# CarbonMatrixLab/AbX

Measured on AMD Instinct MI355X. Metric: diffusion-steps/sec (100 samples, ~350-res complex), higher is better.
Workload: dtype f32; 1 GPU; L352: L=352 (Lab 228 + antigen 124), 100 samples of one complex over 1 GPU(s), 1 step = ScoreNetwork (3 passes) + get_prev + reverse, seeded random weights, ESM off; L=352, samples_total=100, chunk=auto, parallelism=sample-shard x1, no collective in the step

## Files before the change

### abx_amd/csrc/gemm_as.hip

```cpp
#include <stdlib.h>

#include <type_traits>

#include "common.h"
#include "abx_hip.h"

namespace {

typedef __attribute__((address_space(3))) void* lds_ptr_t;
typedef const __attribute__((address_space(1))) void* glb_ptr_t;

constexpr int AS_BM = 64, AS_BN = 128, AS_NK = 12, AS_RING = 3;
constexpr int AS_KT = 4096;
constexpr int AS_A = AS_NK * AS_KT;
constexpr int AS_STAGE = 2 * AS_BN * 32;
constexpr int AS_HALF = AS_KT / 2;
constexpr int AS_OFF_RING = AS_A;
constexpr int AS_OFF_ST = AS_OFF_RING + AS_RING * AS_STAGE;
constexpr int AS_OFF_CONST = AS_OFF_ST + 4 * 64 * 4;
constexpr int AS_LDS = AS_OFF_CONST + 2 * 1024;

__device__ __forceinline__ void as_glds16(const void* src, char* dst_wave_base) {
    __builtin_amdgcn_global_load_lds((glb_ptr_t)src, (lds_ptr_t)dst_wave_base, 16, 0, 0);
}
// ... 552 lines not shown

constexpr int AD_BN = 192, AD_NK2 = 12, AD_NK1 = 8, AD_NS = AD_NK2 + AD_NK1;
constexpr int AD_PLANE = AD_BN * 32;
constexpr int AD_STAGE = 2 * AD_PLANE;
constexpr int AD_OFF_RING = AS_A;
constexpr int AD_OFF_ST = AD_OFF_RING + 2 * AD_STAGE;
constexpr int AD_OFF_CONST = AD_OFF_ST + 4 * 64 * 4;
constexpr int AD_LDS = AD_OFF_CONST + 4 * AD_BN * 4;
static_assert(AD_LDS <= 81920, "two blocks per CU");
constexpr int AD_P0 = 4;
constexpr int ad_wslot(int t) { return t < 4 ? AD_OFF_RING + (t & 1) * AD_STAGE : ((t - 4) % 3 == 0 ? AD_OFF_RING : ((t - 4) % 3 == 1 ? 0 : AD_OFF_RING + AD_STAGE)); }

__device__ __forceinline__ void ad_issue_z(const AbxGemm& g, char* lds, int m0, int b, int wm) {
    const int lane = threadIdx.x & 63;
    const bool remap = g.pair_Lp > 0;
    const long long row0 = remap ? 0 : m0;
    const char* baseA = reinterpret_cast<const char*>(g.A2 + (long long)b * g.sA2b + row0 * g.sA2m);
    unsigned offA[2];
#pragma unroll
    for (int i = 0; i < 2; ++i) {
        const int r = 16 * i + (lane >> 2), p = lane & 3;
        const int kq = p ^ ((r >> 2) & 3);
        const int gri = min(m0 + wm * 32 + r, g.M - 1);
        long long gr = gri;
        if (remap) {
            const int pi = gri / g.pair_Lp, pj = min(gri - pi * g.pair_Lp, g.pair_L - 1);
            gr = (long long)pi * g.pair_L + pj;
        }
        offA[i] = (unsigned)(((gr - row0) * g.sA2m + kq * 4) * 4);
    }
    char* dst = lds + wm * AS_HALF;
#pragma unroll
    for (int kt = 0; kt < AD_NK2; ++kt)
#pragma unroll
        for (int i = 0; i < 2; ++i) as_glds16(baseA + kt * 64 + as_vgpr32(offA[i]), dst + kt * AS_KT + i * 1024);
}

template <bool FIRST>
__device__ __forceinline__ void ad_conv_ptile(AsConv& c, char* img) {
    const int lane = threadIdx.x & 63, r = lane & 31, h = lane >> 5;
    float xv[8];
#pragma unroll
    for (int e = 0; e < 8; ++e) xv[e] = *reinterpret_cast<const float*>(img + (8 * h + e) * 128 + r * 4);
    as_conv_values<FIRST>(c, xv, img);
}

__device__ __forceinline__ void ad_rendezvous(u32x4 (&fa)[2], u32x4 (&fb)[3][2]) {
    asm volatile("s_waitcnt lgkmcnt(0)\n\ts_barrier"
                 : "+v"(fa[0]), "+v"(fa[1]), "+v"(fb[0][0]), "+v"(fb[0][1]), "+v"(fb[1][0]), "+v"(fb[1][1]), "+v"(fb[2][0]), "+v"(fb[2][1])
                 :
                 : "memory");
}
template <int N>
__device__ __forceinline__ void ad_rendezvous_vm(u32x4 (&fa)[2], u32x4 (&fb)[3][2]) {
    asm volatile("s_waitcnt vmcnt(%8) lgkmcnt(0)\n\ts_barrier"
                 : "+v"(fa[0]), "+v"(fa[1]), "+v"(fb[0][0]), "+v"(fb[0][1]), "+v"(fb[1][0]), "+v"(fb[1][1]), "+v"(fb[2][0]), "+v"(fb[2][1])
                 : "n"(N)
                 : "memory");
}

template <bool EDGE>
__device__ __forceinline__ void as_dual_block(const AbxGemm& g, char* lds, int mt, int b) {
    const int lane = threadIdx.x & 63, wave = __builtin_amdgcn_readfirstlane(threadIdx.x >> 6);
    const int wm = wave >> 1, wn = wave & 1, h = lane >> 5;
    const int m0 = mt * AS_BM;
    float* st = reinterpret_cast<float*>(lds + AD_OFF_ST);
    const float* cc = reinterpret_cast<const float*>(lds + AD_OFF_CONST);

    const char* wbase2 = reinterpret_cast<const char*>(g.B2_split);
    const char* wbase1 = reinterpret_cast<const char*>(g.B_split + (long long)b * g.sB3b);
    const long long wk2 = g.sB23k * 2, wk1 = g.sB3k * 2;
    const unsigned wchunk2 = (unsigned)(32 * g.sB23n * 2), wchunk1 = (unsigned)(32 * g.sB3n * 2);
    unsigned woff2, woff1;
    {
        const int row = lane >> 1, half = (lane & 1) ^ ((row >> 3) & 1);
        woff2 = (unsigned)((wm * g.sB23p + (long long)row * g.sB23n + 8 * half) * 2);
        woff1 = (unsigned)((wm * g.sB3p + (long long)row * g.sB3n + 8 * half) * 2);
    }
    auto issue_w = [&](auto s_) __attribute__((always_inline)) {
        constexpr int s = decltype(s_)::value;
        char* dst = lds + ad_wslot(s) + wm * AD_PLANE;
        if constexpr (s < AD_NK2) {
            const char* src = wbase2 + s * wk2;
#pragma unroll
            for (int i = 0; i < 6; ++i) as_glds16(src + i * wchunk2 + as_vgpr32(woff2), dst + i * 1024);
        } else {
            const char* src = wbase1 + (s - AD_NK2) * wk1;
#pragma unroll
            for (int i = 0; i < 6; ++i) as_glds16(src + i * wchunk1 + as_vgpr32(woff1), dst + i * 1024);
        }
    };

    const char* pbase = reinterpret_cast<const char*>(g.A + (long long)b * g.sAb + m0);
    const long long pk = 16LL * g.sAk * 4;
    unsigned poff[2];
#pragma unroll
    for (int i = 0; i < 2; ++i) {
        const int kl = 8 * i + (lane >> 3);
        const int gm = min(m0 + wm * 32 + 4 * (lane & 7), g.M - 4) - m0;
        poff[i] = (unsigned)(((long long)kl * g.sAk + gm) * 4);
    }
    auto issue_p = [&](int kt) __attribute__((always_inline)) {
        char* dst = lds + (AD_P0 + kt) * AS_KT + wm * AS_HALF;
        const char* src = pbase + kt * pk;
#pragma unroll
        for (int i = 0; i < 2; ++i) as_glds16(src + as_vgpr32(poff[i]), dst + i * 1024);
    };

    const float cs2 = __builtin_ldexpf(1.0f, -ABX_F16_A_EXP - g.b2_exp), inv_cs2 = __builtin_ldexpf(1.0f, ABX_F16_A_EXP + g.b2_exp);
    const float cs1 = __builtin_ldexpf(1.0f, -ABX_F16_A_EXP - g.b_exp), inv_cs1 = __builtin_ldexpf(1.0f, ABX_F16_A_EXP + g.b_exp);
    AsConv cz, cp;
    char* a_half = lds + wm * AS_HALF;
    if (wn == 0) {
        ad_issue_z(g, lds, m0, b, wm);
        as_conv_init(cz, g);
        cz.ln = true;
        cz.relu = false;
        cp = cz;
        as_wait_vm<20>();
        as_conv_ktile<true>(cz, a_half);
        as_conv_ktile<false>(cz, a_half + AS_KT);
    } else {
        const float* c0 = wm ? g.ln_csum : g.ln2_csum;
        const float* c1 = wm ? g.bias : g.bias2;
#pragma unroll
        for (int a = 0; a < 2; ++a)
#pragma unroll
            for (int i = 0; i < 3; ++i) {
                char* dst = lds + AD_OFF_CONST + (2 * wm + a) * (AD_BN * 4) + i * 256;
                __builtin_amdgcn_global_load_lds((glb_ptr_t)((a ? c1 : c0) + i * 64 + lane), (lds_ptr_t)dst, 4, 0, 0);
            }
        issue_w(IC<0>{});
        issue_w(IC<1>{});
        as_wait_vm<6>();
    }
    __syncthreads();

    const int offAf = wm * AS_HALF + as_plane_off<32>(0, lane & 31, h);
    const int offBf = as_plane_off<AD_BN>(0, wn * 96 + (lane & 31), h);
    u32x4 fa[2][2], fb[2][3][2];
    auto read_frags = [&](int set, int kt, int wslot) __attribute__((always_inline)) {
#pragma unroll
        for (int p = 0; p < 2; ++p) fa[set][p] = *reinterpret_cast<const u32x4*>(lds + kt * AS_KT + offAf + p * 1024);
#pragma unroll
        for (int j = 0; j < 3; ++j)
#pragma unroll
            for (int p = 0; p < 2; ++p) fb[set][j][p] = *reinterpret_cast<const u32x4*>(lds + offBf + wslot + p * AD_PLANE + j * 1024);
    };

    f32x16 gatev[3], acc[3];
    const float* st_w = st + wm * 32 + 4 * h;
    auto gate_values = [&]() __attribute__((always_inline)) {
#pragma unroll
        for (int j = 0; j < 3; ++j) {
            const int n = wn * 96 + j * 32 + (lane & 31);
            const float csum2 = cc[n] * inv_cs2, bias2 = cc[AD_BN + n];
#pragma unroll
            for (int rq = 0; rq < 4; ++rq) {
                const f32x4 dm4 = *reinterpret_cast<const f32x4*>(st_w + 8 * rq), rs4 = *reinterpret_cast<const f32x4*>(st_w + 64 + 8 * rq);
#pragma unroll
                for (int c = 0; c < 4; ++c) {
                    const float gv = rs4[c] * (gatev[j][4 * rq + c] - dm4[c] * csum2) + bias2;
                    gatev[j][4 * rq + c] = sigmoidf_(gv);
                }
            }
        }
    };

    f32x4 rv[4][3];
    long long row_off_c[4];
    bool row_ok[4];
    auto load_resid = [&]() __attribute__((always_inline)) {
        const float* rd = g.resid + (long long)b * g.sRb;
#pragma unroll
        for (int rq = 0; rq < 4; ++rq) {
            const int m = m0 + wm * 32 + 8 * rq + 4 * h + (lane & 3);
            bool ok = !EDGE || m < g.M;
            long long mo = m;
            if (g.c_pair) {
                const int pi = m / g.pair_Lp, pj = m - pi * g.pair_Lp;
                ok = ok && pj < g.pair_L;
                mo = (long long)pi * g.pair_L + pj;
            }
            row_ok[rq] = ok;
            row_off_c[rq] = mo * g.sCm;
#pragma unroll
            for (int j = 0; j < 3; ++j) {
                const int n = wn * 96 + j * 32 + ((lane & 31) >> 2) * 4;
                rv[rq][j] = (f32x4){0.f, 0.f, 0.f, 0.f};
                if (ok) rv[rq][j] = *reinterpret_cast<const f32x4*>(rd + mo * g.sRm + n);
            }
        }
    };

    auto step = [&](auto s_, auto role_) __attribute__((always_inline)) {
        constexpr int s = decltype(s_)::value, role = decltype(role_)::value, set = s & 1;
        if constexpr (role == 0) ad_rendezvous(fa[set], fb[set]);
        else ad_rendezvous_vm<(s >= 3 && s + 2 < AD_NS) ? 6 : 0>(fa[set], fb[set]);
        if constexpr (role == 1) {
            if constexpr (s < 2) issue_w(IC<s + 2>{});
            else if constexpr (s == 2) { issue_w(IC<4>{}); issue_w(IC<5>{}); }
            else if constexpr (s + 3 < AD_NS) issue_w(IC<s + 3>{});
        } else {
            constexpr int np = s < AD_P0 ? 0 : (s - AD_P0 + 1 < AD_NK1 ? s - AD_P0 + 1 : AD_NK1);
            if constexpr (s >= AD_P0 && s < AD_P0 + AD_NK1) issue_p(s - AD_P0);
            if constexpr (s < AD_NK2 - 2) {
                as_wait_vm<(24 - 2 * (s + 3)) + 2 * np>();
                as_conv_ktile<false>(cz, a_half + (s + 2) * AS_KT);
                if constexpr (s == AD_NK2 - 3) as_conv_finish(cz, st, wm, g.ln_eps, cs2);
            } else if constexpr (s < AD_NK2) {
                as_wait_vm<2 * (np - 1 - (s - 10))>();
                ad_conv_ptile<s == 10>(cp, a_half + (AD_P0 + s - 10) * AS_KT);
            } else if constexpr (s - AD_NK2 + 2 < AD_NK1) {
                constexpr int kp = s - AD_NK2 + 2;
                as_wait_vm<2 * (AD_NK1 - 1 - kp)>();
                ad_conv_ptile<false>(cp, a_half + (AD_P0 + kp) * AS_KT);
                if constexpr (kp == AD_NK1 - 1) as_conv_finish(cp, st + 128, wm, g.ln_eps, cs1, 1.0f / (float)(AD_NK1 * 16));
            }
        }
        if constexpr (s + 1 < AD_NS) read_frags((s + 1) & 1, (s + 1) < AD_NK2 ? s + 1 : s + 1 - AD_NK2 + AD_P0, ad_wslot(s + 1));
        u32x4 p2[3];
#pragma unroll
        for (int j = 0; j < 3; ++j) p2[j] = f16x8_lo(fb[set][j][0]);
        if constexpr (s < AD_NK2) {
            if constexpr (s == 0) {
                const f32x16 z = {0.f, 0.f, 0.f, 0.f, 0.f, 0.f, 0.f, 0.f, 0.f, 0.f, 0.f, 0.f, 0.f, 0.f, 0.f, 0.f};
#pragma unroll
                for (int j = 0; j < 3; ++j) gatev[j] = mfma_split(fa[set][1], p2[j], z);
            } else {
#pragma unroll
                for (int j = 0; j < 3; ++j) gatev[j] = mfma_split(fa[set][1], p2[j], gatev[j]);
            }
#pragma unroll
            for (int j = 0; j < 3; ++j) gatev[j] = mfma_split(fa[set][0], fb[set][j][1], gatev[j]);
#pragma unroll
            for (int j = 0; j < 3; ++j) gatev[j] = mfma_split(fa[set][0], fb[set][j][0], gatev[j]);
        } else {
            if constexpr (s == AD_NK2) {
                const f32x16 z = {0.f, 0.f, 0.f, 0.f, 0.f, 0.f, 0.f, 0.f, 0.f, 0.f, 0.f, 0.f, 0.f, 0.f, 0.f, 0.f};
#pragma unroll
                for (int j = 0; j < 3; ++j) acc[j] = mfma_split(fa[set][1], p2[j], z);
            } else {
#pragma unroll
                for (int j = 0; j < 3; ++j) acc[j] = mfma_split(fa[set][1], p2[j], acc[j]);
            }
#pragma unroll
            for (int j = 0; j < 3; ++j) acc[j] = mfma_split(fa[set][0], fb[set][j][1], acc[j]);
#pragma unroll
            for (int j = 0; j < 3; ++j) acc[j] = mfma_split(fa[set][0], fb[set][j][0], acc[j]);
        }
        if constexpr (s == AD_NK2) gate_values();
    };

    read_frags(0, 0, ad_wslot(0));
    auto walk = [&](auto role_) __attribute__((always_inline)) { as_static_for<0, AD_NS>([&](auto s_) { step(s_, role_); }); };
    if (wn == 0) walk(IC<0>{});
    else walk(IC<1>{});

    float* Cb = g.C + (long long)b * g.sCb;
    bool bad = false;
    load_resid();
#pragma unroll
    for (int j = 0; j < 3; ++j) {
        const int nl = wn * 96 + j * 32 + (lane & 31);
        const float csum1 = cc[2 * AD_BN + nl] * inv_cs1, bias1 = cc[3 * AD_BN + nl];
        const int n = wn * 96 + j * 32 + ((lane & 31) >> 2) * 4;
#pragma unroll
        for (int rq = 0; rq < 4; ++rq) {
            const f32x4 dm4 = *reinterpret_cast<const f32x4*>(st_w + 128 + 8 * rq), rs4 = *reinterpret_cast<const f32x4*>(st_w + 192 + 8 * rq);
            float x[4], o[4];
#pragma unroll
            for (int c = 0; c < 4; ++c) {
                float v = rs4[c] * (acc[j][4 * rq + c] - dm4[c] * csum1);
                v = v + bias1;
                x[c] = v * gatev[j][4 * rq + c];
            }
            as_quad_transpose(x, o);
            f32x4 ov;
#pragma unroll
            for (int c = 0; c < 4; ++c) {
                ov[c] = o[c] + rv[rq][j][c];
                bad |= row_ok[rq] && __builtin_amdgcn_classf(ov[c], 0x207);
            }
            if (row_ok[rq]) *reinterpret_cast<f32x4*>(Cb + row_off_c[rq] + n) = ov;
        }
    }
    if (g.range_flag && __any(bad) && lane == 0) atomicOr(g.range_flag, g.range_tag);
}

__global__ __launch_bounds__(256, 2) void gemm_as_dual_kernel(const AbxGemm g) {
    extern __shared__ __attribute__((aligned(16))) float as_smem[];
    char* lds = reinterpret_cast<char*>(as_smem);
    const ClockProbe probe(g.clock_probe);
    const unsigned ntm = (unsigned)((g.M + AS_BM - 1) / AS_BM);
    const unsigned nwg = gridDim.x, bid = blockIdx.x;
    const unsigned q = nwg >> 3, r = nwg & 7, xcd = bid & 7, loc = bid >> 3;
    const unsigned wgid = (xcd < r ? xcd * (q + 1) : r * (q + 1) + (xcd - r) * q) + loc;
    const int b = (int)(wgid / ntm), mt = (int)(wgid - (unsigned)b * ntm);
    if ((mt + 1) * AS_BM > g.M) as_dual_block<true>(g, lds, mt, b);
    else as_dual_block<false>(g, lds, mt, b);
    probe.finish();
}

int as_dual_dispatch(const AbxGemm& g, hipStream_t st, int* rc) {
    auto al16 = [](const void* p) { return (reinterpret_cast<uintptr_t>(p) & 15) == 0; };
    static const bool off = [] {
        const char* e = getenv("ABX_NO_DUAL_AS");
        return e != nullptr && !(e[0] == '0' && e[1] == 0);
    }();
    if (off) return 1;
    if (g.exact == 1 || g.K != AD_NK1 * 16 || g.K2 != AD_NK2 * 16 || g.N != AD_BN) return 1;
    if (!g.A || g.A_split || g.sAm != 1 || g.M % 4 != 0 || g.M < 4 || !g.B_split || !g.B2_split || !g.b_f16) return 1;
    if (!g.ln_csum || g.ln_stats || !g.ln2_csum || !g.bias || !g.bias2 || !g.resid || !g.C) return 1;
    if (g.act != 0 || g.alpha != 1.0f || g.gate || g.mlp || g.glu || g.rowscale || g.out_ln_w || g.C_split || g.c_transposed || g.a_relu ||
        g.a_pair_transpose > 0 || g.a_pair || g.c_split_tile || g.batch_inner || g.c_planes_from)
        return 1;
    if (!g.c_vec_ok || !g.r_vec_ok) return 1;
    const long long rows_c = g.c_pair ? (long long)g.pair_L * g.pair_L : g.M;
    auto overlaps = [&](const float* p, long long sb, long long sm) {
        const float* c1 = g.C + (g.batch - 1) * g.sCb + (rows_c - 1) * g.sCm + AD_BN;
        const float* p1 = p + (g.batch - 1) * sb + (rows_c - 1) * sm + AD_BN;
        return g.C < p1 && p < c1;
    };
    if (overlaps(g.A2, g.sA2b, g.sA2m) || overlaps(g.resid, g.sRb, g.sRm)) return 1;
    if (!al16(g.A) || g.sAk % 4 != 0 || g.sAb % 4 != 0 || !al16(g.A2) || g.sA2m % 4 != 0 || g.sA2b % 4 != 0) return 1;
    if (!al16(g.B_split) || g.sB3n % 8 != 0 || g.sB3p % 8 != 0 || g.sB3k % 8 != 0 || g.sB3b % 8 != 0) return 1;
    if (!al16(g.B2_split) || g.sB23n % 8 != 0 || g.sB23p % 8 != 0 || g.sB23k % 8 != 0) return 1;
    if (g.b_exp < -100 || g.b_exp > 100 || g.b2_exp < -100 || g.b2_exp > 100) return 1;
    if ((g.pair_Lp > 0 ? (long long)g.pair_L * g.pair_L * g.sA2m : 64LL * g.sA2m) >= (1LL << 30)) return 1;
    if (16LL * g.sAk + g.M >= (1LL << 30)) return 1;
    if (g.sB3p + AD_BN * g.sB3n >= (1LL << 30) || g.sB23p + AD_BN * g.sB23n >= (1LL << 30)) return 1;
    if ((long long)AD_NK1 * g.sB3k >= (1LL << 31) || (long long)AD_NK2 * g.sB23k >= (1LL << 31)) return 1;
    const long long ntm = ((long long)g.M + AS_BM - 1) / AS_BM;
    if (ntm * g.batch >= (1LL << 31)) return 1;
    if (!(g.tune & 16384) && ntm * g.batch < 1024) return 1;
    if (int e = abx_ensure_dynamic_lds(reinterpret_cast<const void*>(&gemm_as_dual_kernel), AD_LDS, "abx_gemm(as, dual)")) {
        *rc = e;
        return 0;
    }
    hipLaunchKernelGGL(gemm_as_dual_kernel, dim3((unsigned)(ntm * g.batch)), dim3(256), AD_LDS, st, g);
    *rc = abx_check_launch("abx_gemm(as, dual)");
    return 0;
}

}

int abx_gemm_as_dispatch(const AbxGemm& g, const AbxGemm* side, hipStream_t st, int* rc) {
    auto al16 = [](const void* p) { return (reinterpret_cast<uintptr_t>(p) & 15) == 0; };
    static const bool off = getenv("ABX_NO_GEMM_AS") != nullptr;
    if (off || (g.tune & 2048)) return 1;
    if (g.A2) return side ? 1 : as_dual_dispatch(g, st, rc);
    if (g.exact == 1 || !g.B_split || !g.b_f16 || g.A_split || !g.A || g.sAk != 1 || g.K != AS_NK * 16) return 1;
    if (g.A2 || g.out_ln_w || g.mlp || g.ln_stats || g.gate || g.resid || g.batch_inner || !g.ln_csum || !g.bias) return 1;
    if (g.act != 0 || g.alpha != 1.0f) return 1;
    if (!al16(g.A) || g.sAm % 4 != 0 || g.sAb % 4 != 0 || !al16(g.B_split) || g.sB3n % 8 != 0 || g.sB3p % 8 != 0 || g.sB3k % 8 != 0) return 1;
    if (g.b_exp < -100 || g.b_exp > 100) return 1;
    if (((g.a_pair_transpose > 0 || g.a_pair) ? (long long)g.M * g.sAm : 64LL * g.sAm) >= (1LL << 30)) return 1;
    if ((long long)(g.K / 16) * g.sB3k >= (1LL << 31)) return 1;
    const long long ntm = ((long long)g.M + AS_BM - 1) / AS_BM;
    if (ntm * g.batch >= (1LL << 31)) return 1;
    if (g.N < 256 || ntm * g.batch < 1024) return 1;
    const bool glu = g.glu != 0;
    if (glu) {
        if (side || !g.C_split || !g.c_split_tile || !g.c_transposed || g.N % 128 != 0 || !g.a_pair || g.pair_Lp <= 0 || g.c_split_L != g.pair_Lp || g.c_split_nA % 32 != 0) return 1;
        if (!g.c_vec_ok || (reinterpret_cast<uintptr_t>(g.C_split) & 15) != 0 || g.sCb % 8 != 0 || g.sCm % 8 != 0 || g.sCk % 8 != 0 || g.sCp % 8 != 0) return 1;
        if (g.sB3b != 0) return 1;
    } else {
        if (g.c_transposed || g.C_split || g.rowscale || g.a_pair_transpose > 0 || g.pair_Lp != 0 || g.batch != 1) return 1;
        if (!g.c_vec_ok || g.N % 64 != 0) return 1;
        if (g.c_planes_from > 0 && (!side || g.c_planes_group != 48 || g.c_planes_from % 32 != 0 || (g.N - g.c_planes_from) % 48 != 0 || g.N >= (1 << 16))) return 1;
        if (side) {
            const AbxGemm& s = *side;
            if (g.N % 128 != 64) return 1;
            if (!s.B_split || !s.b_f16 || s.A_split || s.A != g.A || s.sAk != 1 || s.K != g.K || s.sAm != g.sAm || !s.c_transposed || s.N > 32 ||
                s.exact == 1 || (long long)s.M * s.batch != (long long)g.M || (s.batch > 1 && s.sAb != (long long)s.M * s.sAm) ||
                (s.ln_csum == nullptr) != (g.ln_csum == nullptr) || s.ln_stats || s.gate || s.resid || s.rowscale || s.act != 0 || s.glu || s.C_split ||
                s.A2 || s.out_ln_w || s.mlp || s.a_pair_transpose > 0 || s.pair_Lp != 0 || s.a_relu != g.a_relu ||
                !al16(s.B_split) || s.sB3n % 8 != 0 || s.sB3p % 8 != 0 || s.sB3k % 8 != 0 || s.b_exp < -100 || s.b_exp > 100 ||
                (long long)(s.K / 16) * s.sB3k >= (1LL << 31) || (g.ln_csum && s.ln_eps != g.ln_eps))
                return 1;
        }
    }
    static const AbxGemm none = {};
    const dim3 grid((unsigned)(ntm * g.batch)), block(256);
#define AS_LAUNCH(EPI, SIDE, ABL, ...)                                                                                                   \
    do {                                                                                                                                 \
        if (int e = abx_ensure_dynamic_lds(reinterpret_cast<const void*>(&gemm_as_kernel<EPI, SIDE, ABL, ##__VA_ARGS__>), AS_LDS, "abx_gemm(as)")) { \
            *rc = e;                                                                                                                     \
            return 0;                                                                                                                    \
        }                                                                                                                                \
        hipLaunchKernelGGL((gemm_as_kernel<EPI, SIDE, ABL, ##__VA_ARGS__>), grid, block, AS_LDS, st, g, side ? *side : none);            \
    } while (0)
#ifdef ABX_AS_ABLATE
    const int abl = (g.tune >> 12) & 3;
    if (abl == 1) { if (glu) AS_LAUNCH(AS_EPI_GLU, false, 1); else if (side) AS_LAUNCH(AS_EPI_PLAIN, true, 1); else AS_LAUNCH(AS_EPI_PLAIN, false, 1); }
    else if (abl == 2) { if (glu) AS_LAUNCH(AS_EPI_GLU, false, 2); else if (side) AS_LAUNCH(AS_EPI_PLAIN, true, 2); else AS_LAUNCH(AS_EPI_PLAIN, false, 2); }
    else if (abl == 3) { if (glu) AS_LAUNCH(AS_EPI_GLU, false, 3); else if (side) AS_LAUNCH(AS_EPI_PLAIN, true, 3); else AS_LAUNCH(AS_EPI_PLAIN, false, 3); }
    else
#endif
    if (glu) AS_LAUNCH(AS_EPI_GLU, false, 0);
    else if (side && g.c_planes_from > 0) AS_LAUNCH(AS_EPI_PLAIN, true, 0, true);
    else if (side) AS_LAUNCH(AS_EPI_PLAIN, true, 0);
    else AS_LAUNCH(AS_EPI_PLAIN, false, 0);
#undef AS_LAUNCH
    *rc = abx_check_launch("abx_gemm(as)");
    return 0;
}
```

### abx_amd/ops.py

```python
import ctypes as C
import math

import torch

from abx_amd import _lib
from abx_amd._lib import (AbxGemm, AbxTriAttn, AbxIpaTail, AbxHeadsTail, AbxScoreArgs, AbxReverseArgs, AbxGuidanceArgs, AbxDesignScoreArgs, AbxRelaxArgs, AbxInterfaceArgs, AbxDistogramArgs, AbxEnsemblePairsArgs, AbxEnsembleClusterArgs, AbxLinearPack, AbxLinearSrc,
                           AbxTriMulPack, AbxTriAttnPack, AbxTriRowPack, check)


def _stream():
    return C.c_void_p(torch.cuda.current_stream().cuda_stream)


def _p(t):
    if t is None:
        return None
    assert t.is_cuda, 'libabx_hip works on device memory only'
    return t.data_ptr()


def _f32(t):
    assert t.dtype == torch.float32, t.dtype
    return t


GEMM_TUNE = int(__import__('os').environ.get('ABX_GEMM_TUNE', '0'))

RANGE_TAGS = {'gemm': 1, 'contraction': 2, 'plane_projection': 4, 'tri_mul_tail': 8, 'pair_transition': 16, 'ipa_pair_init': 32,
              'tri_attn': 64, 'ipa_tail': 128, 'heads_tail': 256, 'gemm_late': 512}
RANGE_CHECK = not bool(__import__('os').environ.get('ABX_NO_RANGE_CHECK'))
_range_words = {}


RANGE_SLOTS = 4
RANGE_SLOT = 0


def range_words(device):
    idx = torch.device(device).index
    idx = torch.cuda.current_device() if idx is None else idx
    w = _range_words.get(idx)
    if w is None:
        w = torch.zeros(RANGE_SLOTS, dtype=torch.int32, device=torch.device('cuda', idx))
        _range_words[idx] = w
    return w


def range_word(device):
    return range_words(device)[0:1]


def range_ptr(device):
    return range_words(device).data_ptr() + 4 * RANGE_SLOT


def range_names(bits):
    return [n for n, b in RANGE_TAGS.items() if bits & b]


RANGE_ORDER = ('gemm', 'plane_projection', 'contraction', 'tri_mul_tail', 'tri_attn', 'pair_transition', 'ipa_pair_init', 'gemm_late', 'ipa_tail', 'heads_tail')


def first_range_tag(bits, skip=0):
    for n in RANGE_ORDER:
        if bits & RANGE_TAGS[n] & ~skip:
            return RANGE_TAGS[n]
    return 0


GEMM_EXACT = False


def gemm_kernel_name(M, N, K, batch, a_kcontig=True, b_ncontig=True, transposed=False, split=False, exact=None, a_split=False, dual=False, out_ln=False):
    b = lambda x: 'true' if x else 'false'
    if dual:
        tune = GEMM_TUNE or 0
        if (not GEMM_EXACT and int(exact or 0) != 1 and not (tune & 2048) and N == 192 and K == 128 and not a_kcontig and M % 4 == 0
                and not transposed and split and (((M + 63) // 64) * batch >= 1024 or (tune & 16384))):
            return 'gemm_as_dual_kernel'
        return 'gemm3_dual_kernel<128, 96, 32, 96, 3>'
    if out_ln:
        return 'gemm3_oln_kernel<128, 128, 32, 128, 4>'
    exact = 1 if GEMM_EXACT else int(exact or 0)
    blocks128 = ((M + 127) // 128) * ((N + 127) // 128) * batch
    wide192 = ((N + 191) // 192) * 192 <= ((N + 127) // 128) * 128
    if exact != 1 and split and N <= 32 and a_kcontig and not a_split and K % 16 == 0:
        return f'gemm3_kernel<128, 32, 32, 32, 0, {b(transposed)}, 6>'
    if exact != 1 and split and N > 64 and (blocks128 >= 256 or exact == 2) and K % 16 == 0 and (a_kcontig or a_split or M % 4 == 0):
        amode = 2 if a_split else (0 if a_kcontig else 1)
        pad128, pad192 = ((N + 127) // 128) * 128, ((N + 191) // 192) * 192
        wide = pad192 <= pad128 if a_split else (wide192 and N % 128 != 0)
        cfg = (128, 192, 32, 192, 3) if wide else (128, 128, 32, 128, 4)
        if not wide and blocks128 < 384 and M > 64:
            cfg = (64, 128, 32, 64, 4)
        return f'gemm3_kernel<{cfg[0]}, {cfg[1]}, {cfg[2]}, {cfg[3]}, {amode}, {b(transposed)}, {cfg[4]}>'
    if N <= 32:
        cfg = (128, 32, 32, 32, 3)
    elif N <= 64:
        cfg = (128, 64, 32, 64, 3)
    elif blocks128 < 512:
        cfg = (64, 64, 32, 32, 3)
    elif wide192:
        cfg = (128, 192, 64, 96, 2)
    else:
        cfg = (128, 128, 64, 64, 3)
    return f'gemm_kernel<{cfg[0]}, {cfg[1]}, {cfg[2]}, {cfg[3]}, 16, {b(a_kcontig)}, {b(b_ncontig)}, {b(transposed)}, {cfg[4]}>'


def gemm_as_kernel_name(g, side=None):
    if GEMM_EXACT or (g.tune & 2048) or g.exact == 1 or not g.B_split or not g.b_f16 or g.A_split or not g.A or g.sAk != 1 or g.K != 192:
        return None
    if g.A2 or g.out_ln_w or g.mlp or g.ln_stats or g.gate or g.resid or g.batch_inner or not g.ln_csum or not g.bias or g.act != 0 or g.alpha != 1.0:
        return None
    ntm = (g.M + 63) // 64
    if g.N < 256 or ntm * g.batch < 1024:
        return None
    if g.glu:
        if side is not None or not g.C_split or not g.c_split_tile or not g.c_transposed or g.N % 128 != 0 or not g.a_pair or g.pair_Lp <= 0:
            return None
        return 'gemm_as_kernel<1, false, 0, false>'
    if g.c_transposed or g.C_split or g.rowscale or g.a_pair_transpose > 0 or g.pair_Lp != 0 or g.batch != 1 or g.N % 64 != 0:
        return None
    if side is not None:
        s2 = side
        if g.N % 128 != 64 or not s2.B_split or not s2.c_transposed or s2.N > 32 or s2.K != g.K or s2.M * s2.batch != g.M or s2.act != 0 or s2.exact == 1:
            return None
        return 'gemm_as_kernel<0, true, 0, true>' if g.c_planes_from > 0 else 'gemm_as_kernel<0, true, 0, false>'
    return 'gemm_as_kernel<0, false, 0, false>'


SPLIT_MIN_L = 64


def gemm_mode(L):
    return 1 if (GEMM_EXACT or L < SPLIT_MIN_L) else 2


def gemm_split_eligible(M, N, K, batch=1):
    return (not GEMM_EXACT) and N > 64 and K % 16 == 0 and ((M + 127) // 128) * ((N + 127) // 128) * batch >= 256


def pack_glu_weights(Wv, Wg, bv=None, bg=None):
    K, C_ = Wv.shape
    assert Wg.shape == (K, C_) and C_ % 64 == 0
    W = torch.stack([Wv.reshape(K, C_ // 32, 32), Wg.reshape(K, C_ // 32, 32)], dim=2).reshape(K, 2 * C_).contiguous()
    b = None
    if bv is not None or bg is not None:
        z = torch.zeros(C_, device=Wv.device, dtype=Wv.dtype)
        b = torch.stack([(bv if bv is not None else z).reshape(C_ // 32, 32), (bg if bg is not None else z).reshape(C_ // 32, 32)],
                        dim=1).reshape(2 * C_).contiguous()
    return W, b


_PERM16 = (0, 1, 2, 3, 8, 9, 10, 11, 4, 5, 6, 7, 12, 13, 14, 15)


def permute_k16(Wt):
    K, N = Wt.shape
    assert K % 16 == 0
    idx = torch.tensor(_PERM16, device=Wt.device)
    return Wt.reshape(K // 16, 16, N)[:, idx, :].reshape(K, N).contiguous()


class WeightPlanes(torch.Tensor):
    w_exp = 0
    __torch_function__ = torch._C._disabled_torch_function_impl


def split_weights(Wt):
    K, N = Wt.shape
    _f32(Wt)
    Kp = (K + 15) // 16 * 16
    amax = float(Wt.abs().max())
    if not math.isfinite(amax):
        raise ValueError('split_weights: non-finite weight')
    w_exp = 14 - math.frexp(amax)[1] if amax > 0 else 0
    w_exp = max(-100, min(100, w_exp))
    out = torch.empty(Kp // 16, 2, N, 16, device=Wt.device, dtype=torch.float16)
    check(_lib.load().abx_split_weights_f16(_p(Wt), Wt.stride(1), Wt.stride(0), N, K, w_exp, _p(out), _stream()), 'abx_split_weights_f16')
    out = out.as_subclass(WeightPlanes)
    out.w_exp = w_exp
    return out


def weights_to_float(w3):
    v = (w3[:, 0].float() + w3[:, 1].float()) * 2.0 ** (-w3.w_exp)
    return v.permute(0, 2, 1).reshape(-1, w3.shape[2])


def _weight_planes(w3, N, K=None, what='B3'):
    assert isinstance(w3, WeightPlanes) and w3.dtype == torch.float16 and w3.is_contiguous() and w3.shape[1:] == (2, N, 16), \
        f'{what}: WeightPlanes (ops.split_weights) of N = {N} expected'
    assert K is None or w3.shape[0] * 16 >= K
    return w3


def gemm(A, B, Cout, *, ln=None, a_relu=False, bias=None, alpha=1.0, act=0, rowscale=None, gate=None, gate_sigmoid=True,
         resid=None, tune=None, B3=None, exact=None, a_pair_transpose=0, glu=False, pair=None, a_pair=False, c_pair=False, dual=None, out_ln=None, clock_probe=None, mlp=None, c_split_nA=0, c_split_tile=False,
         defer=False, range_class=None, c_plane_cols=None):
    lib = _lib.load()
    g = AbxGemm()
    a_planes, b_planes, c_planes = A.dtype == torch.int16, B.dtype == torch.int16, Cout.dtype == torch.int16
    if a_planes and A.dim() == 6:
        assert B.dtype == torch.int16 and B.dim() == 6 and B.shape[:2] == A.shape[:2]
        g.batch_inner, g.sA3i, g.sB3i = A.shape[1], A.stride(1), B.stride(1)
        bo_a, bo_b = A.stride(0), B.stride(0)
        A = A.as_strided((A.shape[0] * A.shape[1],) + tuple(A.shape[2:]), (0,) + tuple(A.stride()[2:]), A.storage_offset())
        B = B.as_strided((B.shape[0] * B.shape[1],) + tuple(B.shape[2:]), (0,) + tuple(B.stride()[2:]), B.storage_offset())
    else:
        bo_a = bo_b = None
    if a_planes:
        assert A.dim() == 5 and A.shape[2] == 2 and A.shape[4] == 16 and A.stride(4) == 1
        nb, KT, _, M, _ = A.shape
        K = KT * 16
        g.A_split, g.sA3b, g.sA3k, g.sA3p, g.sA3m = _p(A), (A.stride(0) if nb > 1 else 0), A.stride(1), A.stride(2), A.stride(3)
        if bo_a is not None:
            g.sA3b = bo_a
    else:
        if A.dim() == 2:
            A = A.unsqueeze(0)
        nb, M, K = A.shape
        _f32(A)
        g.A, g.sAb, g.sAm, g.sAk = _p(A), A.stride(0) if nb > 1 else 0, A.stride(1), A.stride(2)
        if a_pair:
            assert pair is not None and M == pair[0] * pair[0], (A.shape, pair)
            M = pair[0] * pair[1]
            if c_split_tile:
                M = ((pair[0] + 7) // 8 * 8) * ((pair[1] + 15) // 16 * 16)
    if b_planes:
        assert B.dim() == 5 and B.shape[2] == 2 and B.shape[4] == 16 and B.stride(4) == 1 and B.shape[1] * 16 == K and B.shape[0] == nb
        N = B.shape[3]
        g.B_split, g.sB3b, g.sB3k, g.sB3p, g.sB3n = _p(B), (B.stride(0) if nb > 1 else 0), B.stride(1), B.stride(2), B.stride(3)
        if bo_b is not None:
            g.sB3b = bo_b
    else:
        if B.dim() == 2:
            B = B.unsqueeze(0)
        assert B.shape[1] == K, (A.shape, B.shape)
        N = B.shape[2]
        _f32(B)
        g.B, g.sBb, g.sBk, g.sBn = _p(B), (B.stride(0) if B.shape[0] > 1 else 0), B.stride(1), B.stride(2)
    No = N // 2 if glu else N
    if mlp is not None:
        B32m, bias2m = mlp
        No = B32m.shape[2]
        _weight_planes(B32m, No, what='mlp B3_2')
        assert B32m.shape[0] * 16 == N
        g.mlp, g.N2, g.b2_exp = (2 if gate is not None else 1), No, B32m.w_exp
        g.B2_split, g.sB23k, g.sB23p, g.sB23n = _p(B32m), B32m.stride(0), B32m.stride(1), B32m.stride(2)
        g.bias2 = _p(bias2m)
        assert act == (2 if gate is not None else 1) and ln is not None and ln[0] is None
    if c_planes:
        L = Cout.shape[4]
        Lp = pair[1] if pair is not None else L
        assert Cout.dim() == 6 and Cout.shape == (nb, No, (Lp + 15) // 16, 2, L, 16) and (c_split_tile or M == L * Lp), (Cout.shape, nb, M, N)
        assert not c_split_tile or (a_pair and pair is not None), 'c_split_tile: the A rows come through the pair-row map (a_pair, pair=(L, Lp))'
        assert Cout.stride(5) == 1 and Cout.stride(4) == 16
        g.C_split, g.sCb, g.sCm, g.sCk, g.sCp, g.c_split_L = _p(Cout), (Cout.stride(0) if nb > 1 else 0), Cout.stride(1), Cout.stride(2), Cout.stride(3), Lp
        g.c_transposed, g.c_split_nA, g.c_split_tile = 1, int(c_split_nA), int(bool(c_split_tile))
    else:
        if Cout.dim() == 2:
            Cout = Cout.unsqueeze(0)
        assert Cout.shape == (nb, pair[0] * pair[0] if c_pair else M, No), (Cout.shape, (nb, M, No))
        _f32(Cout)
        g.C = _p(Cout)
        Cl = Cout
        g.sCb = Cl.stride(0) if nb > 1 else 0
        if Cl.stride(2) == 1:
            g.c_transposed, g.sCm = 0, Cl.stride(1)
        else:
            assert Cl.stride(1) == 1, 'Cout must be n-contiguous or m-contiguous'
            g.c_transposed, g.sCm = 1, Cl.stride(2)
    g.M, g.N, g.K, g.batch = M, N, K, nb
    g.a_pair_transpose = int(a_pair_transpose)
    if pair is not None:
        g.pair_L, g.pair_Lp, g.a_pair, g.c_pair = int(pair[0]), int(pair[1]), int(bool(a_pair)), int(bool(c_pair))
        assert c_split_tile or M == pair[0] * pair[1], (M, pair)
    g.glu = int(bool(glu))
    if ln is not None:
        stats, csum = ln
        assert csum.numel() == N
        g.ln_csum, g.ln_eps = _p(_f32(csum)), 1e-5
        if stats is not None:
            assert stats.numel() == 2 * nb * M, (stats.shape, nb, M)
            g.ln_stats, g.sSb = _p(_f32(stats)), M
    g.a_relu = 1 if a_relu else 0
    g.exact = 1 if GEMM_EXACT else int(exact or 0)
    if B3 is not None:
        _weight_planes(B3, N, K)
        assert not a_planes, 'weight planes go with an fp32 A (the plane x plane contraction takes activation images on both sides)'
        g.B_split, g.sB3k, g.sB3p, g.sB3n, g.sB3b = _p(B3), B3.stride(0), B3.stride(1), B3.stride(2), 0
        g.b_f16, g.b_exp = 1, B3.w_exp
    g.tune = GEMM_TUNE if tune is None else tune
    if c_plane_cols is not None:
        g.c_planes_from, g.c_planes_group = int(c_plane_cols[0]), int(c_plane_cols[1])
    if RANGE_CHECK and g.exact != 1:
        g.range_flag = range_ptr(Cout.device)
        g.range_tag = RANGE_TAGS[('tri_attn' if gate is not None else 'pair_transition') if mlp is not None else 'tri_mul_tail' if dual is not None else 'ipa_pair_init' if out_ln is not None
                                 else 'plane_projection' if c_planes else 'contraction' if a_planes else (range_class or 'gemm')]
    if dual is not None:
        A2, B32, csum2, bias2 = dual
        if A2.dim() == 2:
            A2 = A2.unsqueeze(0)
        _f32(A2)
        assert A2.stride(2) == 1 and A2.shape[0] == nb and A2.shape[1] == (pair[0] * pair[0] if pair is not None else M)
        K2 = A2.shape[2]
        _weight_planes(B32, N, what='dual B3_2')
        assert B32.shape[0] * 16 == K2 and csum2.numel() == N
        g.b2_exp = B32.w_exp
        g.A2, g.sA2b, g.sA2m, g.K2 = _p(A2), (A2.stride(0) if nb > 1 else 0), A2.stride(1), K2
        g.B2_split, g.sB23k, g.sB23p, g.sB23n = _p(B32), B32.stride(0), B32.stride(1), B32.stride(2)
        g.ln2_csum, g.bias2 = _p(_f32(csum2)), _p(bias2)
        if g.ln_eps == 0:
            g.ln_eps = 1e-5
    if out_ln is not None:
        assert out_ln[0].numel() == N and out_ln[1].numel() == N
        g.out_ln_w, g.out_ln_b = _p(_f32(out_ln[0])), _p(_f32(out_ln[1]))
        g.out_ln_eps = float(out_ln[2]) if len(out_ln) > 2 else 1e-5
    if clock_probe is not None:
        assert clock_probe.dtype == torch.int64 and clock_probe.numel() >= 2
        g.clock_probe = _p(clock_probe)
    g.bias = _p(bias)
    g.alpha = float(alpha)
    g.act = int(act)
    if rowscale is not None:
        rs_rows = pair[0] * pair[1] if c_split_tile else M
        assert rowscale.numel() == nb * rs_rows and rowscale.is_contiguous()
        g.rowscale, g.sRSb = _p(_f32(rowscale)), rs_rows
    if gate is not None:
        if gate.dim() == 2:
            gate = gate.unsqueeze(0)
        cd, sd = (1, 2) if g.c_transposed else (2, 1)
        assert gate.shape == (nb, M if c_planes else Cout.shape[1], N) and gate.stride(cd) == 1, 'gate must be laid out like Cout (mlp: (M, N) rows)'
        g.gate, g.sGb, g.sGm, g.gate_sigmoid = _p(_f32(gate)), (gate.stride(0) if nb > 1 else 0), gate.stride(sd), int(gate_sigmoid)
    if resid is not None:
        if resid.dim() == 2:
            resid = resid.unsqueeze(0)
        cd, sd = (1, 2) if g.c_transposed else (2, 1)
        assert resid.shape == (nb, M if c_planes else Cout.shape[1], No if mlp is not None else N) and resid.stride(cd) == 1, 'resid must be laid out like Cout'
        g.resid, g.sRb, g.sRm = _p(_f32(resid)), (resid.stride(0) if nb > 1 else 0), resid.stride(sd)
    if defer:
        return g
    check(lib.abx_gemm(C.byref(g), _stream()), 'abx_gemm')
    return Cout


def gemm_side(g_main, g_side):
    check(_lib.load().abx_gemm_side(C.byref(g_main), C.byref(g_side), _stream()), 'abx_gemm_side')


def planes_to_float(p, a_side, dim=0):
    h = p.view(torch.float16).float()
    p0, p1 = h.select(dim, 0), h.select(dim, 1)
    return (p0 + p1 / 2048.0) * 16.0 if a_side else (p0 + p1) / 16.0


def row_stats(x, out=None, eps=1e-5):
    lib = _lib.load()
    _f32(x)
    if x.dim() == 2:
        rows, K = x.shape
        assert x.stride(1) == 1
        if out is None:
            out = torch.empty(rows, 2, device=x.device, dtype=torch.float32)
        check(lib.abx_row_stats(_p(x), 0, x.stride(0), 1, 1, rows, K, eps, _p(out), _stream()), 'abx_row_stats')
    else:
        nb, rows, K = x.shape
        assert x.stride(1) == 1, 'channel-major layout expected'
        if out is None:
            out = torch.empty(nb * rows, 2, device=x.device, dtype=torch.float32)
        check(lib.abx_row_stats(_p(x), x.stride(0), 1, x.stride(2), nb, rows, K, eps, _p(out), _stream()), 'abx_row_stats')
    return out


def layernorm(x, gamma, beta, out=None, res=None, eps=1e-5):
    lib = _lib.load()
    rows, K = x.shape
# ... 826 lines not shown
```

Baseline: 173.8 sample-steps/s.

## Add fused async-LDS MLP kernel for 192→768→192 transition GEMMs

Adds a new gemm_as_mlp kernel that fuses layernorm-folded first GEMM, ReLU, and second GEMM with residual add for the K=192, N=768, N2=192 transition MLP. Weights stream through a global_load_lds ring buffer, and the hidden activations stay in registers chunk by chunk, so no intermediate is written to memory. The two wave columns split the hidden chunks and reduce their partial output sums through LDS at the end. This adds a large specialised code path with tight dispatch conditions and an env opt-out.

```diff
diff --git a/abx_amd/csrc/gemm_as.hip b/abx_amd/csrc/gemm_as.hip
--- a/abx_amd/csrc/gemm_as.hip
+++ b/abx_amd/csrc/gemm_as.hip
@@ -878,6 +878,290 @@
     probe.finish();
 }
 
+constexpr int AM_NC = 6, AM_STEPS = 24, AM_NH = AM_NC * 128, AM_N2 = 192;
+constexpr int AM_OFF_RING = AS_A;
+constexpr int AM_OFF_ST = AM_OFF_RING + AS_RING * AS_STAGE;
+constexpr int AM_OFF_CONST = AM_OFF_ST + 2 * 64 * 4;
+constexpr int AM_LDS = AM_OFF_CONST + 2 * AM_NH * 4;
+static_assert(AM_LDS <= 81920, "two blocks per CU");
+static_assert(4 * 3 * 16 * 64 * 4 <= AS_A, "the partial sums of the four waves meet in the A region");
+
+template <bool WITH_A>
+__device__ __forceinline__ void am_rendezvous(u32x4 (&fa)[2], u32x4 (&fb)[2][2]) {
+    if constexpr (WITH_A) as_rendezvous_free(fa, fb);
+    else asm volatile("s_waitcnt lgkmcnt(0)\n\ts_barrier" : "+v"(fb[0][0]), "+v"(fb[0][1]), "+v"(fb[1][0]), "+v"(fb[1][1]) : : "memory");
+}
+template <bool WITH_A>
+__device__ __forceinline__ void am_rendezvous_vm(u32x4 (&fa)[2], u32x4 (&fb)[2][2]) {
+    if constexpr (WITH_A) as_rendezvous<4>(fa, fb);
+    else asm volatile("s_waitcnt vmcnt(4) lgkmcnt(0)\n\ts_barrier" : "+v"(fb[0][0]), "+v"(fb[0][1]), "+v"(fb[1][0]), "+v"(fb[1][1]) : : "memory");
+}
+
+template <bool EDGE>
+__device__ __forceinline__ void as_mlp_block(const AbxGemm& g, char* lds, int mt, int b) {
+    const int lane = threadIdx.x & 63, wave = __builtin_amdgcn_readfirstlane(threadIdx.x >> 6);
+    const int wm = wave >> 1, wn = wave & 1, h = lane >> 5;
+    const int m0 = mt * AS_BM;
+    float* st = reinterpret_cast<float*>(lds + AM_OFF_ST);
+    float* cst = reinterpret_cast<float*>(lds + AM_OFF_CONST);
+
+    const char* w1base = reinterpret_cast<const char*>(g.B_split + (long long)b * g.sB3b);
+    const char* w2base = reinterpret_cast<const char*>(g.B2_split);
+    constexpr long long w1k = 2LL * AM_NH * 16 * 2, w2k = 2LL * AM_N2 * 16 * 2;
+    constexpr long long w1chunk = 32 * 16 * 2, w2chunk = 32 * 16 * 2;
+    unsigned w1off, w2off;
+    {
+        const int row = lane >> 1, half = (lane & 1) ^ ((row >> 3) & 1);
+        w1off = (unsigned)((wm * (AM_NH * 16) + row * 16 + 8 * half) * 2);
+        w2off = (unsigned)((wm * (AM_N2 * 16) + row * 16 + 8 * half) * 2);
+    }
+    auto issue_w = [&](int c, auto s_) __attribute__((always_inline)) {
+        constexpr int s = decltype(s_)::value;
+        char* dst = lds + AM_OFF_RING + (s % AS_RING) * AS_STAGE + wm * 4096;
+        const int cc = min(c, AM_NC - 1);
+        if constexpr (s < AS_NK) {
+            const char* src = w1base + s * w1k + (long long)cc * 4 * w1chunk;
+#pragma unroll
+            for (int i = 0; i < 4; ++i) as_glds16(src + i * w1chunk + as_vgpr32(w1off), dst + i * 1024);
+        } else {
+            constexpr int kk = (s - AS_NK) / 3, t = (s - AS_NK) % 3;
+#pragma unroll
+            for (int i = 0; i < 4; ++i) {
+                const char* src = w2base + (long long)(cc * 8 + 4 * (i >> 1) + kk) * w2k + (2 * t + (i & 1)) * w2chunk;
+                as_glds16(src + as_vgpr32(w2off), dst + i * 1024);
+            }
+        }
+    };
+
+    const float cs = __builtin_ldexpf(1.0f, -ABX_F16_A_EXP - g.b_exp), inv_cs = __builtin_ldexpf(1.0f, ABX_F16_A_EXP + g.b_exp);
+    char* a_half = lds + wm * AS_HALF;
+    if (wn == 0) {
+        AsConv cv;
+        as_issue_a(g, lds, m0, b, wm);
+        as_conv_init(cv, g);
+        as_static_for<0, AS_NK>([&](auto kt_) {
+            constexpr int kt = decltype(kt_)::value;
+            as_wait_vm<2 * (AS_NK - 1 - kt)>();
+            as_conv_ktile<kt == 0>(cv, a_half + kt * AS_KT);
+        });
+        as_conv_finish(cv, st, wm, g.ln_eps, cs);
+    } else {
+        for (int i = wm * 64 + lane; i < AM_NH; i += 128) {
+            cst[i] = g.ln_csum[i] * inv_cs;
+            cst[AM_NH + i] = g.bias[i];
+        }
+        asm volatile("" ::: "memory");
+        issue_w(0, IC<0>{});
+        issue_w(0, IC<1>{});
+        issue_w(0, IC<2>{});
+        as_wait_vm<8>();
+    }
+    __syncthreads();
+
+    const float dm = st[wm * 32 + (lane & 31)], rs = st[64 + wm * 32 + (lane & 31)];
+
+    const int offAf = wm * AS_HALF + as_plane_off<32>(0, lane & 31, h);
+    const int offBf = AM_OFF_RING + as_plane_off<AS_BN>(0, wn * 64 + (lane & 31), h);
+    u32x4 fa[2][2], fb[2][2][2];
+    auto read_frags = [&](auto s_) __attribute__((always_inline)) {
+        constexpr int s = decltype(s_)::value, set = s & 1;
+        if constexpr (s < AS_NK) {
+#pragma unroll
+            for (int p = 0; p < 2; ++p) fa[set][p] = *reinterpret_cast<const u32x4*>(lds + s * AS_KT + offAf + p * 1024);
+        }
+#pragma unroll
+        for (int j = 0; j < 2; ++j)
+#pragma unroll
+            for (int p = 0; p < 2; ++p)
+                fb[set][j][p] = *reinterpret_cast<const u32x4*>(lds + offBf + (s % AS_RING) * AS_STAGE + p * (AS_BN * 32) + j * 1024);
+    };
+
+    f32x16 acc1[2], acc2[6];
+#pragma unroll
+    for (int t = 0; t < 6; ++t)
+#pragma unroll
+        for (int r = 0; r < 16; ++r) acc2[t][r] = 0.f;
+    u32x4 hf[2];
+
+    auto step = [&](int c, auto s_, auto role_) __attribute__((always_inline)) {
+        constexpr int s = decltype(s_)::value, role = decltype(role_)::value, set = s & 1;
+        if constexpr (role == 0) am_rendezvous<(s < AS_NK)>(fa[set], fb[set]);
+        else am_rendezvous_vm<(s < AS_NK)>(fa[set], fb[set]);
+        if constexpr (role == 1) {
+            if constexpr (s + 3 < AM_STEPS) issue_w(c, IC<s + 3>{});
+            else issue_w(c + 1, IC<s + 3 - AM_STEPS>{});
+        }
+        read_frags(IC<(s + 1) % AM_STEPS>{});
+        __builtin_amdgcn_sched_barrier(0);
+        if constexpr (s < AS_NK) {
+            u32x4 p2[2];
+#pragma unroll
+            for (int j = 0; j < 2; ++j) p2[j] = f16x8_lo(fb[set][j][0]);
+            if constexpr (s == 0) {
+                const f32x16 z = {0.f, 0.f, 0.f, 0.f, 0.f, 0.f, 0.f, 0.f, 0.f, 0.f, 0.f, 0.f, 0.f, 0.f, 0.f, 0.f};
+#pragma unroll
+                for (int j = 0; j < 2; ++j) acc1[j] = mfma_split(p2[j], fa[set][1], z);
+            } else {
+#pragma unroll
+                for (int j = 0; j < 2; ++j) acc1[j] = mfma_split(p2[j], fa[set][1], acc1[j]);
+            }
+#pragma unroll
+            for (int j = 0; j < 2; ++j) acc1[j] = mfma_split(fb[set][j][1], fa[set][0], acc1[j]);
+#pragma unroll
+            for (int j = 0; j < 2; ++j) acc1[j] = mfma_split(fb[set][j][0], fa[set][0], acc1[j]);
+        } else {
+            constexpr int kk = (s - AS_NK) / 3, t = (s - AS_NK) % 3;
+            if constexpr (t == 0) {
+                constexpr int j = kk >> 1, s2 = kk & 1;
+                float v[8];
+#pragma unroll
+                for (int q = 0; q < 2; ++q) {
+                    const int hc = c * 128 + role * 64 + j * 32 + 8 * (2 * s2 + q) + 4 * h;
+                    const f32x4 cs4 = *reinterpret_cast<const f32x4*>(cst + hc), bi4 = *reinterpret_cast<const f32x4*>(cst + AM_NH + hc);
+#pragma unroll
+                    for (int e = 0; e < 4; ++e) {
+                        const float x = rs * (acc1[j][8 * s2 + 4 * q + e] - dm * cs4[e]) + bi4[e];
+                        v[4 * q + e] = relu_keep_nan(x);
+                    }
+                }
+                unsigned q0[4], q1[4];
+#pragma unroll
+                for (int e = 0; e < 4; ++e) split2b(v[2 * e], v[2 * e + 1], q0[e], q1[e]);
+                hf[0] = u32x4{q0[0], q0[1], q0[2], q0[3]};
+                hf[1] = u32x4{q1[0], q1[1], q1[2], q1[3]};
+            }
+#pragma unroll
+            for (int j = 0; j < 2; ++j) acc2[2 * t + j] = mfma_split(hf[1], fb[set][j][0], acc2[2 * t + j]);
+#pragma unroll
+            for (int j = 0; j < 2; ++j) acc2[2 * t + j] = mfma_split(hf[0], fb[set][j][1], acc2[2 * t + j]);
+#pragma unroll
+            for (int j = 0; j < 2; ++j) acc2[2 * t + j] = mfma_split(hf[0], fb[set][j][0], acc2[2 * t + j]);
+        }
+    };
+
+    read_frags(IC<0>{});
+    auto walk = [&](auto role_) __attribute__((always_inline)) {
+#pragma unroll 1
+        for (int c = 0; c < AM_NC; ++c) as_static_for<0, AM_STEPS>([&](auto s_) { step(c, s_, role_); });
+    };
+    if (wn == 0) walk(IC<0>{});
+    else walk(IC<1>{});
+
+    f32x4 rv[4][3];
+    long long row_off_c[4];
+    bool row_ok[4];
+    {
+        const float* rd = g.resid + (long long)b * g.sRb;
+#pragma unroll
+        for (int rq = 0; rq < 4; ++rq) {
+            const int m = m0 + wm * 32 + 8 * rq + 4 * h + (lane & 3);
+            row_ok[rq] = !EDGE || m < g.M;
+            row_off_c[rq] = (long long)m * g.sCm;
+#pragma unroll
+            for (int j = 0; j < 3; ++j) {
+                const int n = wn * 96 + j * 32 + ((lane & 31) >> 2) * 4;
+                rv[rq][j] = (f32x4){0.f, 0.f, 0.f, 0.f};
+                if (row_ok[rq]) rv[rq][j] = *reinterpret_cast<const f32x4*>(rd + (long long)m * g.sRm + n);
+            }
+        }
+    }
+    asm volatile("s_waitcnt vmcnt(0)" ::: "memory");
+    __syncthreads();
+    float* xch = reinterpret_cast<float*>(lds);
+    f32x16 sum[3];
+    if (wn == 0) {
+#pragma unroll
+        for (int t = 0; t < 3; ++t)
+#pragma unroll
+            for (int r = 0; r < 16; ++r) xch[((wm * 2 + 1) * 3 + t) * 1024 + r * 64 + lane] = acc2[3 + t][r];
+    } else {
+#pragma unroll
+        for (int t = 0; t < 3; ++t)
+#pragma unroll
+            for (int r = 0; r < 16; ++r) xch[((wm * 2 + 0) * 3 + t) * 1024 + r * 64 + lane] = acc2[t][r];
+    }
+    __syncthreads();
+    if (wn == 0) {
+#pragma unroll
+        for (int t = 0; t < 3; ++t)
+#pragma unroll
+            for (int r = 0; r < 16; ++r) sum[t][r] = acc2[t][r] + xch[((wm * 2 + 0) * 3 + t) * 1024 + r * 64 + lane];
+    } else {
+#pragma unroll
+        for (int t = 0; t < 3; ++t)
+#pragma unroll
+            for (int r = 0; r < 16; ++r) sum[t][r] = xch[((wm * 2 + 1) * 3 + t) * 1024 + r * 64 + lane] + acc2[3 + t][r];
+    }
+
+    const float cs2 = __builtin_ldexpf(1.0f, -4 - g.b2_exp);
+    float* Cb = g.C + (long long)b * g.sCb;
+    bool bad = false;
+#pragma unroll
+    for (int j = 0; j < 3; ++j) {
+        const float bias2 = g.bias2 ? g.bias2[wn * 96 + j * 32 + (lane & 31)] : 0.f;
+        const int n = wn * 96 + j * 32 + ((lane & 31) >> 2) * 4;
+#pragma unroll
+        for (int rq = 0; rq < 4; ++rq) {
+            float x[4], o[4];
+#pragma unroll
+            for (int c = 0; c < 4; ++c) x[c] = sum[j][4 * rq + c] * cs2 + bias2;
+            as_quad_transpose(x, o);
+            f32x4 ov;
+#pragma unroll
+            for (int c = 0; c < 4; ++c) {
+                ov[c] = o[c] + rv[rq][j][c];
+                bad |= row_ok[rq] && __builtin_amdgcn_classf(ov[c], 0x207);
+            }
+            if (row_ok[rq]) *reinterpret_cast<f32x4*>(Cb + row_off_c[rq] + n) = ov;
+        }
+    }
+    if (g.range_flag && __any(bad) && lane == 0) atomicOr(g.range_flag, g.range_tag);
+}
+
+__global__ __launch_bounds__(256, 2) void gemm_as_mlp_kernel(const AbxGemm g) {
+    extern __shared__ __attribute__((aligned(16))) float as_smem[];
+    char* lds = reinterpret_cast<char*>(as_smem);
+    const ClockProbe probe(g.clock_probe);
+    const unsigned ntm = (unsigned)((g.M + AS_BM - 1) / AS_BM);
+    const unsigned nwg = gridDim.x, bid = blockIdx.x;
+    const unsigned q = nwg >> 3, r = nwg & 7, xcd = bid & 7, loc = bid >> 3;
+    const unsigned wgid = (xcd < r ? xcd * (q + 1) : r * (q + 1) + (xcd - r) * q) + loc;
+    const int b = (int)(wgid / ntm), mt = (int)(wgid - (unsigned)b * ntm);
+    if ((mt + 1) * AS_BM > g.M) as_mlp_block<true>(g, lds, mt, b);
+    else as_mlp_block<false>(g, lds, mt, b);
+    probe.finish();
+}
+
+int as_mlp_dispatch(const AbxGemm& g, hipStream_t st, int* rc) {
+    auto al16 = [](const void* p) { return (reinterpret_cast<uintptr_t>(p) & 15) == 0; };
+    static const bool off = [] {
+        const char* e = getenv("ABX_NO_MLP_AS");
+        return e != nullptr && !(e[0] == '0' && e[1] == 0);
+    }();
+    if (off || (g.tune & 48)) return 1;
+    if (g.mlp != 1 || g.act != 1 || g.K != AS_NK * 16 || g.N != AM_NH || g.N2 != AM_N2 || g.exact == 1) return 1;
+    if (!g.A || g.A_split || g.sAk != 1 || !g.ln_csum || g.ln_stats || !g.bias || !g.B_split || !g.b_f16 || !g.B2_split || !g.C || !g.resid) return 1;
+    if (g.alpha != 1.0f || g.gate || g.rowscale || g.glu || g.A2 || g.out_ln_w || g.C_split || g.c_transposed || g.a_relu || g.a_pair_transpose > 0 ||
+        g.a_pair || g.pair_Lp != 0 || g.c_pair || g.c_split_tile || g.batch_inner || g.c_planes_from)
+        return 1;
+    if (!g.c_vec_ok || !g.r_vec_ok) return 1;
+    if (!al16(g.A) || g.sAm % 4 != 0 || g.sAb % 4 != 0) return 1;
+    if (!al16(g.B_split) || g.sB3b % 8 != 0) return 1;
+    if (!al16(g.B2_split)) return 1;
+    if (g.sB3n != 16 || g.sB3p != AM_NH * 16 || g.sB3k != 2LL * AM_NH * 16 || g.sB23n != 16 || g.sB23p != AM_N2 * 16 || g.sB23k != 2LL * AM_N2 * 16) return 1;
+    if (g.b_exp < -100 || g.b_exp > 100 || g.b2_exp < -100 || g.b2_exp > 100) return 1;
+    if (g.sAm < 0 || 64LL * g.sAm >= (1LL << 30)) return 1;
+    const long long ntm = ((long long)g.M + AS_BM - 1) / AS_BM;
+    if (ntm * g.batch >= (1LL << 31)) return 1;
+    if (int e = abx_ensure_dynamic_lds(reinterpret_cast<const void*>(&gemm_as_mlp_kernel), AM_LDS, "abx_gemm(as, mlp)")) {
+        *rc = e;
+        return 0;
+    }
+    hipLaunchKernelGGL(gemm_as_mlp_kernel, dim3((unsigned)(ntm * g.batch)), dim3(256), AM_LDS, st, g);
+    *rc = abx_check_launch("abx_gemm(as, mlp)");
+    return 0;
+}
+
 int as_dual_dispatch(const AbxGemm& g, hipStream_t st, int* rc) {
     auto al16 = [](const void* p) { return (reinterpret_cast<uintptr_t>(p) & 15) == 0; };
     static const bool off = [] {
@@ -926,6 +1210,7 @@
     static const bool off = getenv("ABX_NO_GEMM_AS") != nullptr;
     if (off || (g.tune & 2048)) return 1;
     if (g.A2) return side ? 1 : as_dual_dispatch(g, st, rc);
+    if (g.mlp == 1) return side ? 1 : as_mlp_dispatch(g, st, rc);
     if (g.exact == 1 || !g.B_split || !g.b_f16 || g.A_split || !g.A || g.sAk != 1 || g.K != AS_NK * 16) return 1;
     if (g.A2 || g.out_ln_w || g.mlp || g.ln_stats || g.gate || g.resid || g.batch_inner || !g.ln_csum || !g.bias) return 1;
     if (g.act != 0 || g.alpha != 1.0f) return 1;
diff --git a/abx_amd/ops.py b/abx_amd/ops.py
--- a/abx_amd/ops.py
+++ b/abx_amd/ops.py
@@ -71,8 +71,19 @@
 GEMM_EXACT = False
 
 
-def gemm_kernel_name(M, N, K, batch, a_kcontig=True, b_ncontig=True, transposed=False, split=False, exact=None, a_split=False, dual=False, out_ln=False):
+def gemm_kernel_name(M, N, K, batch, a_kcontig=True, b_ncontig=True, transposed=False, split=False, exact=None, a_split=False, dual=False, out_ln=False,
+                     mlp=False, N2=0, tune=None):
     b = lambda x: 'true' if x else 'false'
+    if mlp:
+        tune = (GEMM_TUNE or 0) if tune is None else int(tune)
+        if tune & 32:
+            return 'gemm3_mlp3_kernel'
+        if tune & 16:
+            return 'gemm3_mlp_kernel<1>'
+        if (not GEMM_EXACT and int(exact or 0) != 1 and not (tune & 2048) and K == 192 and N == 768 and N2 == 192 and a_kcontig and not transposed
+                and split):
+            return 'gemm_as_mlp_kernel'
+        return 'gemm3_mlp_kernel<2>'
     if dual:
         tune = GEMM_TUNE or 0
         if (not GEMM_EXACT and int(exact or 0) != 1 and not (tune & 2048) and N == 192 and K == 128 and not a_kcontig and M % 4 == 0
```

Measured after the change: 175.0 sample-steps/s (median of 6 runs). Within noise of the previous version (+0.7%).
